# helmholtz-analytics/mpi4torch

Hardware: AMD Instinct MI355X
Metric: allreduce_fwdbwd_algbw_GBps (higher is better)
Workload: dtype bf16; 1 GPU; model=allreduce_1GiB_bf16_fwd_bwd, parallelism=dp1

## Files before the change

csrc/ops.cpp:

```cpp

#include "ops.hpp"
#include "transport.hpp"
#include "kernels.hpp"

#include <torch/csrc/autograd/function.h>
#include <torch/csrc/autograd/functions/utils.h>
#include <torch/csrc/autograd/variable.h>
#include <ATen/core/TensorBody.h>
#include <ATen/WrapDimUtils.h>

#include <ATen/hip/impl/HIPStreamMasqueradingAsCUDA.h>

#include <algorithm>
#include <cstdlib>
#include <cstring>
#include <functional>
#include <limits>
#include <map>
#include <mutex>
#include <tuple>

namespace m4a {

using at::Tensor;
using torch::autograd::Node;
using torch::autograd::variable_list;


Communicator::Communicator(std::string group_name)
    : group_name_(std::move(group_name)) {}

int64_t Communicator::GetRank() { return cpu_tr().rank(); }
int64_t Communicator::GetSize() { return cpu_tr().size(); }

Transport& Communicator::cpu_tr() {
  std::lock_guard<std::mutex> g(mu_);
  if (!cpu_tr_) {
    cpu_tr_ = group_name_.empty() ? make_local_transport()
                                  : make_c10d_transport(group_name_);
  }
  return *cpu_tr_;
}

Transport& Communicator::gpu_tr(int device) {
  std::lock_guard<std::mutex> g(mu_);
  if (!gpu_tr_) {
    if (group_name_.empty()) {
      if (!cpu_tr_) cpu_tr_ = make_local_transport();
      return *cpu_tr_;
    }
    gpu_tr_ = make_rccl_transport(group_name_, device);
    gpu_device_ = device;
  }
  TORCH_CHECK(device == gpu_device_,
              "mpi4torch_amd: one GPU per process (torchrun model); "
              "communicator bound to device ", gpu_device_,
              " but got a tensor on device ", device);
  return *gpu_tr_;
}

Transport& Communicator::tr_for(const Tensor& t) {
  if (t.is_cuda() && !config().force_host_staging) {
    return gpu_tr((int)t.get_device());
  }
  return cpu_tr();
}

namespace {

struct DeviceStager {
  explicit DeviceStager(const Tensor& t)
      : orig_device_(t.device()),
        active_(t.is_cuda() && config().force_host_staging) {}
  Tensor to_comm(const Tensor& t) const {
    return active_ ? t.to(at::kCPU) : t;
  }
  Tensor from_comm(Tensor t) const {
    return active_ ? t.to(orig_device_) : std::move(t);
  }
  at::Device orig_device_;
  bool active_;
};


struct AxisGeom {
  int64_t before = 1, axis = 0, after = 1, after_b = 0, esize = 0;
};

AxisGeom axis_geom(const Tensor& t, int64_t axis) {
  AxisGeom g;
  auto sizes = t.sizes();
  for (int64_t i = 0; i < axis; ++i) g.before *= sizes[i];
  g.axis = sizes[axis];
  for (int64_t i = axis + 1; i < (int64_t)sizes.size(); ++i)
    g.after *= sizes[i];
  g.esize = t.element_size();
  g.after_b = g.after * g.esize;
  return g;
}

hipStream_t current_gpu_stream(const Tensor& t) {
  return c10::hip::getCurrentHIPStreamMasqueradingAsCUDA((int)t.get_device())
      .stream();
}

void move_axis_blocks(const Tensor& full, int64_t axis,
                      const std::vector<int64_t>& displs,
                      const std::vector<int64_t>& counts,
                      std::vector<Tensor>& blocks, bool pack,
                      int64_t row_lo = 0, int64_t row_hi = -1) {
  const auto g = axis_geom(full, axis);
  if (row_hi < 0) row_hi = g.before;
  const int64_t rows = row_hi - row_lo;
  if (rows <= 0) return;
  if (full.is_cuda()) {
    std::vector<SlabDesc> descs;
    descs.reserve(counts.size());
    char* base = static_cast<char*>(full.data_ptr());
    for (size_t i = 0; i < counts.size(); ++i) {
      if (counts[i] == 0 || g.before * g.after == 0) continue;
      char* bp = static_cast<char*>(blocks[i].data_ptr());
      SlabDesc d;
      d.before = rows;
      d.count = counts[i];
      d.after_b = g.after_b;
      if (pack) {
        d.src = base + displs[i] * g.after_b + row_lo * g.axis * g.after_b;
        d.src_pitch_b = g.axis * g.after_b;
        d.dst = bp + row_lo * counts[i] * g.after_b;
        d.dst_pitch_b = counts[i] * g.after_b;
      } else {
        d.src = bp + row_lo * counts[i] * g.after_b;
        d.src_pitch_b = counts[i] * g.after_b;
        d.dst = base + displs[i] * g.after_b + row_lo * g.axis * g.after_b;
        d.dst_pitch_b = g.axis * g.after_b;
      }
      descs.push_back(d);
    }
    if (!descs.empty()) {
      launch_slab_copy(descs.data(), (int)descs.size(),
                       current_gpu_stream(full));
    }
  } else {
    if (g.before * g.after == 0) return;
    auto f3 = full.view({g.before, g.axis, g.after})
                  .narrow(0, row_lo, rows);
    for (size_t i = 0; i < counts.size(); ++i) {
      if (counts[i] == 0) continue;
      auto b3 = blocks[i].view({g.before, counts[i], g.after})
                    .narrow(0, row_lo, rows);
      if (pack) {
        b3.copy_(f3.narrow(1, displs[i], counts[i]));
      } else {
        f3.narrow(1, displs[i], counts[i]).copy_(b3);
      }
    }
  }
}


Tensor fast_clone(const Tensor& in) {
  if (!in.is_cuda() || in.numel() == 0) return in.clone();
  auto out = at::empty_like(in);
  SlabDesc d;
  d.src = in.data_ptr();
  d.dst = out.data_ptr();
  d.before = 1;
  d.count = 1;
  d.after_b = in.numel() * in.element_size();
  d.src_pitch_b = d.after_b;
  d.dst_pitch_b = d.after_b;
  launch_slab_copy(&d, 1, current_gpu_stream(in));
  return out;
}

std::vector<int64_t> prefix_displs(const std::vector<int64_t>& counts) {
  std::vector<int64_t> d(counts.size(), 0);
  for (size_t i = 1; i < counts.size(); ++i) d[i] = d[i - 1] + counts[i - 1];
  return d;
}

int64_t phase_count(const Tensor& t, int64_t per_rank_bytes) {
  const int64_t c = config().pipeline_chunk_bytes;
  if (c <= 0) return 1;
  if (t.is_cuda()) {
    hipStreamCaptureStatus st = hipStreamCaptureStatusNone;
    (void)hipStreamIsCapturing(current_gpu_stream(t), &st);
    if (st != hipStreamCaptureStatusNone) return 1;
  }
  return std::min<int64_t>(
      4, std::max<int64_t>(1, (per_rank_bytes + c - 1) / c));
}

void phased_funnel_exchange(
    Transport& tr, int64_t K, int64_t rows,
    const std::vector<Tensor>& sblocks, const std::vector<int>& speers,
    const std::vector<int64_t>& srowe, std::vector<Tensor>& rblocks,
    const std::vector<int>& rpeers, const std::vector<int64_t>& rrowe,
    const std::function<void(int64_t, int64_t)>& pack_phase,
    const std::function<void(int64_t, int64_t)>& unpack_phase) {
  auto bound = [&](int64_t k) { return rows * k / K; };
  auto slice = [](const Tensor& blk, int64_t lo, int64_t len) {
    auto flat = blk.view({-1});
    return len > 0 ? flat.narrow(0, lo, len) : flat.narrow(0, 0, 0);
  };
  std::vector<uint64_t> reqs((size_t)K);
  for (int64_t k = 0; k < K; ++k) {
    const int64_t b0 = bound(k), b1 = bound(k + 1);
    if (pack_phase) pack_phase(b0, b1);
    std::vector<Tensor> sk(sblocks.size()), rk(rblocks.size());
    for (size_t i = 0; i < sblocks.size(); ++i) {
      sk[i] = slice(sblocks[i], b0 * srowe[i], (b1 - b0) * srowe[i]);
    }
    for (size_t j = 0; j < rblocks.size(); ++j) {
      rk[j] = slice(rblocks[j], b0 * rrowe[j], (b1 - b0) * rrowe[j]);
    }
    reqs[(size_t)k] = tr.iexchange(sk, speers, rk, rpeers);
  }
  for (int64_t k = 0; k < K; ++k) {
    wait_request(reqs[(size_t)k]);
    if (unpack_phase) unpack_phase(bound(k), bound(k + 1));
  }
}


bool is_logical(int64_t op) { return op == kLAnd || op == kLOr || op == kLXor; }
bool is_bitwise(int64_t op) { return op == kBAnd || op == kBOr || op == kBXor; }
bool is_arith(int64_t op) {
  return op == kSum || op == kProd || op == kMin || op == kMax;
}

struct SigHash {
  size_t h;
  explicit SigHash(const char* opname) : h(std::hash<std::string>()(opname)) {}
  void mix(int64_t v) {
    h ^= std::hash<int64_t>()(v) + 0x9e3779b97f4a7c15ull + (h << 6) + (h >> 2);
  }
};

void debug_compare_sig(const std::string& group, const char* opname,
                       SigHash& sig) {
  auto all =
      host_allgather_int64(group, (int64_t)(sig.h & 0x7fffffffffffffffll));
  for (size_t r = 1; r < all.size(); ++r) {
    TORCH_CHECK(all[r] == all[0],
                "mpi4torch_amd[debug]: collective desync detected at ", opname,
                " — rank ", r, " issued a different op/shape/dtype/arguments "
                "than rank 0. This would deadlock without "
                "MPI4TORCH_AMD_DEBUG=1.");
  }
}

void debug_check_collective(const std::string& group, const char* opname,
                            const at::Tensor& t,
                            std::initializer_list<int64_t> args) {
  if (!config().debug_collectives || group.empty()) return;
  SigHash sig(opname);
  sig.mix((int64_t)t.scalar_type());
  for (auto s : t.sizes()) sig.mix(s);
  for (auto a : args) sig.mix(a);
  debug_compare_sig(group, opname, sig);
}

void debug_check_axis_collective(const std::string& group, const char* opname,
                                 const at::Tensor& t,
                                 std::initializer_list<int64_t> axes,
                                 std::initializer_list<int64_t> args) {
  if (!config().debug_collectives || group.empty()) return;
  SigHash sig(opname);
  sig.mix((int64_t)t.scalar_type());
  sig.mix(t.dim());
  for (int64_t i = 0; i < t.dim(); ++i) {
    bool skip = false;
    for (auto a : axes) skip = skip || a == i;
    sig.mix(skip ? -1 : t.size(i));
  }
  for (auto a : args) sig.mix(a);
  debug_compare_sig(group, opname, sig);
}

void debug_check_dtype_collective(const std::string& group,
                                  const char* opname, at::ScalarType dtype,
                                  std::initializer_list<int64_t> args) {
  if (!config().debug_collectives || group.empty()) return;
  SigHash sig(opname);
  sig.mix((int64_t)dtype);
  for (auto a : args) sig.mix(a);
  debug_compare_sig(group, opname, sig);
}

void check_op(int64_t op) {
  TORCH_CHECK(op >= kMax && op <= kMaxLoc, "invalid reduction op ", op);
}

bool is_pairloc(int64_t op) { return op == kMinLoc || op == kMaxLoc; }

bool native_reduce_dtype(const Transport& tr, at::ScalarType t) {
  if (tr.is_gpu()) {
    switch (t) {
      case at::kByte:
      case at::kChar:
      case at::kInt:
      case at::kLong:
      case at::kHalf:
      case at::kFloat:
      case at::kDouble:
      case at::kBFloat16:
        return true;
      case at::kFloat8_e4m3fn:
      case at::kFloat8_e5m2: {
        static const bool want_native = []() {
          const char* e = std::getenv("MPI4TORCH_AMD_NATIVE_FP8");
          return e && e[0] == '1';
        }();
        return want_native &&
               const_cast<Transport&>(tr).fp8_reduce_supported(t);
      }
      default:
        return false;
    }
  }
  switch (t) {
    case at::kByte:
    case at::kChar:
    case at::kInt:
// ... 1765 lines not shown
  }();
  attach_history(result, grad_fn);
  return result;
}


namespace {
struct AlltoallvBackward : public M4ANode {
  AlltoallvBackward(int64_t gaxis, int64_t saxis,
                    std::vector<int64_t> tgt, std::vector<int64_t> src)
      : gaxis(gaxis), saxis(saxis), tgt(std::move(tgt)),
        src(std::move(src)) {}
  std::string name() const override { return "M4AAlltoallvBackward"; }
  variable_list apply(variable_list&& grads) override {
    variable_list out(1);
    if (should_compute_output(0)) {
      out[0] = comm->Alltoallv(grads[0], saxis, gaxis, tgt, src);
    }
    return out;
  }
  int64_t gaxis, saxis;
  std::vector<int64_t> tgt, src;
};

struct AlltoallBackward : public M4ANode {
  AlltoallBackward(int64_t gaxis, int64_t saxis, int64_t numelem)
      : gaxis(gaxis), saxis(saxis), numelem(numelem) {}
  std::string name() const override { return "M4AAlltoallBackward"; }
  variable_list apply(variable_list&& grads) override {
    variable_list out(1);
    if (should_compute_output(0)) {
      out[0] = comm->Alltoall(grads[0], saxis, gaxis, numelem);
    }
    return out;
  }
  int64_t gaxis, saxis, numelem;
};

}

Tensor Communicator::AlltoallvImpl(const Tensor& input, int64_t gatheraxis,
                                   int64_t scatteraxis, int64_t numelem,
                                   const std::vector<int64_t>& target_counts,
                                   const std::vector<int64_t>& source_sizes) {
  gatheraxis = at::maybe_wrap_dim(gatheraxis, input.dim());
  scatteraxis = at::maybe_wrap_dim(scatteraxis, input.dim());
  const bool explicit_counts = !target_counts.empty();
  std::shared_ptr<M4ANode> grad_fn;
  if (torch::autograd::compute_requires_grad(input)) {
    if (explicit_counts) {
      grad_fn = make_node<AlltoallvBackward>(
          c10::intrusive_ptr<Communicator>::unsafe_reclaim_from_nonowning(this),
          gatheraxis, scatteraxis, source_sizes, target_counts);
    } else {
      grad_fn = make_node<AlltoallBackward>(
          c10::intrusive_ptr<Communicator>::unsafe_reclaim_from_nonowning(this),
          gatheraxis, scatteraxis, input.size(gatheraxis));
    }
    grad_fn->set_next_edges(torch::autograd::collect_next_edges(input));
  }
  auto result = [&]() {
    at::AutoDispatchBelowADInplaceOrView guard;
    DeviceStager stager(input);
    auto in = stager.to_comm(input).contiguous().variable_data();
    auto& tr = tr_for(in);
    if (w1_shortcut(tr)) {
      const int64_t want = explicit_counts ? target_counts[0] : numelem;
      TORCH_CHECK(want == in.size(scatteraxis),
                  "Alltoall: numelem must equal the scatter-axis size at "
                  "world size 1");
      return stager.from_comm(fast_clone(in));
    }
    const int me = tr.rank();
    const int P = tr.size();
    debug_check_axis_collective(group_name_, "Alltoall", in,
                                {gatheraxis, scatteraxis},
                                {gatheraxis, scatteraxis, explicit_counts});

    std::vector<int64_t> scounts;
    if (explicit_counts) {
      TORCH_CHECK((int)target_counts.size() == P,
                  "Alltoallv: target_counts must have world_size entries");
      TORCH_CHECK((int)source_sizes.size() == P,
                  "Alltoallv: source_sizes must have world_size entries");
      scounts = target_counts;
    } else {
      scounts = host_allgather_int64(group_name_, numelem);
    }
    auto sdispls = prefix_displs(scounts);

    std::vector<int64_t> s_offs(P), s_lens(P);
    std::vector<int64_t> r_offs(P), r_lens(P);
    std::vector<int64_t> outsizes = in.sizes().vec();
    int64_t send_axis = scatteraxis, recv_axis = gatheraxis;
    std::vector<int64_t> srcsz;

    if (gatheraxis != scatteraxis) {
      const int64_t stotal = sdispls.back() + scounts.back();
      TORCH_CHECK(in.size(scatteraxis) == stotal,
                  "Alltoall: scatter-axis size (", in.size(scatteraxis),
                  ") must equal the sum of per-rank numelem (", stotal, ")");
      auto gsizes = explicit_counts
                        ? source_sizes
                        : host_allgather_int64(group_name_,
                                               in.size(gatheraxis));
      TORCH_CHECK(gsizes[me] == in.size(gatheraxis),
                  "Alltoallv: source_sizes[rank] must equal the local "
                  "gather-axis size");
      auto gdispls = prefix_displs(gsizes);
      for (int j = 0; j < P; ++j) {
        s_offs[j] = sdispls[j];
        s_lens[j] = scounts[j];
        r_offs[j] = gdispls[j];
        r_lens[j] = gsizes[j];
      }
      outsizes[gatheraxis] = gdispls.back() + gsizes.back();
      outsizes[scatteraxis] = scounts[me];
      srcsz = gsizes;
    } else {
      auto nsizes = explicit_counts
                        ? source_sizes
                        : host_allgather_int64(group_name_,
                                               in.size(gatheraxis));
      TORCH_CHECK(nsizes[me] == in.size(gatheraxis),
                  "Alltoallv: source_sizes[rank] must equal the local "
                  "axis size");
      auto ndispls = prefix_displs(nsizes);
      const int64_t totaln = ndispls.back() + nsizes.back();
      const int64_t totalm = sdispls.back() + scounts.back();
      TORCH_CHECK(totaln == totalm,
                  "Alltoall (same axis): global axis length mismatch (",
                  totaln, " vs ", totalm, ")");
      const int64_t my_lo = ndispls[me], my_hi = my_lo + nsizes[me];
      const int64_t tgt_lo = sdispls[me], tgt_hi = tgt_lo + scounts[me];
      for (int j = 0; j < P; ++j) {
        const int64_t slo = std::max(my_lo, sdispls[j]);
        const int64_t shi = std::min(my_hi, sdispls[j] + scounts[j]);
        s_offs[j] = slo - my_lo;
        s_lens[j] = std::max<int64_t>(0, shi - slo);
        const int64_t rlo = std::max(ndispls[j], tgt_lo);
        const int64_t rhi = std::min(ndispls[j] + nsizes[j], tgt_hi);
        r_offs[j] = rlo - tgt_lo;
        r_lens[j] = std::max<int64_t>(0, rhi - rlo);
      }
      outsizes[gatheraxis] = scounts[me];
      srcsz = nsizes;
    }

    auto out = at::empty(outsizes, in.options());
    const auto gs = axis_geom(in, send_axis);
    const auto gr = axis_geom(out, recv_axis);
    const bool send_packed = gs.before != 1;
    const bool recv_packed = gr.before != 1;
    auto sblocks = make_blocks(in, gs.before, gs.after, s_lens, s_offs, &in);
    auto rblocks = make_blocks(out, gr.before, gr.after, r_lens, r_offs, &out);
    auto peers = iota_peers(P);

    int64_t send_before_shared = 1, recv_before_shared = 1;
    {
      const int64_t src_max =
          *std::max_element(srcsz.begin(), srcsz.end());
      const int64_t sc_max =
          *std::max_element(scounts.begin(), scounts.end());
      auto insz = in.sizes();
      for (int64_t d = 0; d < send_axis; ++d) {
        send_before_shared *=
            (d == recv_axis && send_axis != recv_axis) ? src_max : insz[d];
      }
      for (int64_t d = 0; d < recv_axis; ++d) {
        recv_before_shared *= (d == scatteraxis && send_axis != recv_axis)
                                  ? sc_max
                                  : outsizes[d];
      }
    }
    const bool send_m = send_before_shared > 1;
    const bool recv_m = recv_before_shared > 1;
    int64_t K = 1;
    if ((send_m || recv_m) &&
        (send_axis == recv_axis || send_m != recv_m)) {
      int64_t global_elems = 1;
      for (size_t d = 0; d < outsizes.size(); ++d) {
        global_elems *= (d == (size_t)scatteraxis)
                            ? (sdispls.back() + scounts.back())
                            : outsizes[d];
      }
      K = phase_count(in, global_elems / P * in.element_size());
    }

    if (K > 1) {
      const int me_ = me;
      auto send_geom = [&](int j) -> std::pair<int64_t, int64_t> {
        if (send_axis == recv_axis || send_m) {
          return {gs.before, s_lens[j] * gs.after};
        }
        int64_t before = 1, after = 1;
        for (int64_t d = 0; d < (int64_t)outsizes.size(); ++d) {
          const int64_t sz =
              (d == scatteraxis) ? scounts[j] : outsizes[d];
          if (d < recv_axis) before *= sz;
          else if (d > recv_axis) after *= sz;
        }
        return {before, srcsz[me_] * after};
      };
      auto recv_geom = [&](int i) -> std::pair<int64_t, int64_t> {
        if (send_axis == recv_axis || recv_m) {
          return {gr.before, r_lens[i] * gr.after};
        }
        int64_t before = 1, after = 1;
        auto insz = in.sizes();
        for (int64_t d = 0; d < (int64_t)insz.size(); ++d) {
          const int64_t sz = (d == recv_axis) ? srcsz[i] : insz[d];
          if (d < send_axis) before *= sz;
          else if (d > send_axis) after *= sz;
        }
        return {before, scounts[me_] * after};
      };
      auto bound = [&](int64_t rows, int64_t k) { return rows * k / K; };
      auto slice = [](const Tensor& blk, int64_t lo, int64_t len) {
        auto flat = blk.view({-1});
        return len > 0 ? flat.narrow(0, lo, len) : flat.narrow(0, 0, 0);
      };
      std::vector<uint64_t> reqs((size_t)K);
      for (int64_t k = 0; k < K; ++k) {
        if (send_packed) {
          move_axis_blocks(in, send_axis, s_offs, s_lens, sblocks, true,
                           bound(gs.before, k), bound(gs.before, k + 1));
        }
        std::vector<Tensor> sk(P), rk(P);
        for (int j = 0; j < P; ++j) {
          auto sg = send_geom(j);
          sk[j] = slice(sblocks[j], bound(sg.first, k) * sg.second,
                        (bound(sg.first, k + 1) - bound(sg.first, k)) *
                            sg.second);
          auto rg = recv_geom(j);
          rk[j] = slice(rblocks[j], bound(rg.first, k) * rg.second,
                        (bound(rg.first, k + 1) - bound(rg.first, k)) *
                            rg.second);
        }
        reqs[(size_t)k] = tr.iexchange(sk, peers, rk, peers);
      }
      for (int64_t k = 0; k < K; ++k) {
        wait_request(reqs[(size_t)k]);
        if (recv_packed) {
          move_axis_blocks(out, recv_axis, r_offs, r_lens, rblocks, false,
                           bound(gr.before, k), bound(gr.before, k + 1));
        }
      }
      return stager.from_comm(std::move(out));
    }

    if (send_packed) {
      move_axis_blocks(in, send_axis, s_offs, s_lens, sblocks, true);
    }
    tr.exchange(sblocks, peers, rblocks, peers);
    if (recv_packed) {
      move_axis_blocks(out, recv_axis, r_offs, r_lens, rblocks,
                       false);
    }
    return stager.from_comm(std::move(out));
  }();
  attach_history(result, grad_fn);
  return result;
}

Tensor Communicator::Alltoall(const Tensor& input, int64_t gatheraxis,
                              int64_t scatteraxis, int64_t numelem) {
  return AlltoallvImpl(input, gatheraxis, scatteraxis, numelem, {}, {});
}

Tensor Communicator::Alltoallv(const Tensor& input, int64_t gatheraxis,
                               int64_t scatteraxis,
                               std::vector<int64_t> target_counts,
                               std::vector<int64_t> source_sizes) {
  TORCH_CHECK(!target_counts.empty(),
              "Alltoallv: target_counts must not be empty");
  return AlltoallvImpl(input, gatheraxis, scatteraxis,
                       -1, target_counts, source_sizes);
}



namespace {
struct AlltoallPairwiseBackward : public M4ANode {
  AlltoallPairwiseBackward(int64_t axis, std::vector<int64_t> send,
                           std::vector<int64_t> recv)
      : axis(axis), send(std::move(send)), recv(std::move(recv)) {}
  std::string name() const override { return "M4AAlltoallPairwiseBackward"; }
  variable_list apply(variable_list&& grads) override {
    variable_list out(1);
    if (should_compute_output(0)) {
      out[0] = comm->AlltoallPairwise(grads[0], axis, recv, send);
    }
    return out;
  }
  int64_t axis;
  std::vector<int64_t> send, recv;
};
}

Tensor Communicator::AlltoallPairwise(const Tensor& input, int64_t axis,
                                      std::vector<int64_t> send_counts,
                                      std::vector<int64_t> recv_counts) {
  axis = at::maybe_wrap_dim(axis, input.dim());
  auto& tr0 = cpu_tr();
  const int P = tr0.size();
  TORCH_CHECK((int)send_counts.size() == P,
              "AlltoallPairwise: send_counts must have world_size entries");
  if (recv_counts.empty() && P > 1) {
    auto mat = host_allgather_int64_vec(group_name_, send_counts);
    recv_counts.resize(P);
    const int me = tr0.rank();
    for (int j = 0; j < P; ++j) recv_counts[j] = mat[(int64_t)j * P + me];
  }
  if (P == 1 && recv_counts.empty()) recv_counts = send_counts;
  TORCH_CHECK((int)recv_counts.size() == P,
              "AlltoallPairwise: recv_counts must have world_size entries");

  std::shared_ptr<M4ANode> grad_fn;
  if (torch::autograd::compute_requires_grad(input)) {
    grad_fn = make_node<AlltoallPairwiseBackward>(
        c10::intrusive_ptr<Communicator>::unsafe_reclaim_from_nonowning(this),
        axis, send_counts, recv_counts);
    grad_fn->set_next_edges(torch::autograd::collect_next_edges(input));
  }
  auto result = [&]() {
    at::AutoDispatchBelowADInplaceOrView guard;
    DeviceStager stager(input);
    auto in = stager.to_comm(input).contiguous().variable_data();
    auto& tr = tr_for(in);
    auto s_displs = prefix_displs(send_counts);
    auto r_displs = prefix_displs(recv_counts);
    const int64_t s_total = s_displs.back() + send_counts.back();
    const int64_t r_total = r_displs.back() + recv_counts.back();
    TORCH_CHECK(in.size(axis) == s_total,
                "AlltoallPairwise: sum of send_counts (", s_total,
                ") must equal the axis size (", in.size(axis), ")");
    auto outsizes = in.sizes().vec();
    outsizes[axis] = r_total;
    auto out = at::empty(outsizes, in.options());
    if (tr.size() == 1 && !config().force_full_path) {
      out.copy_(in);
      return stager.from_comm(std::move(out));
    }
    debug_check_axis_collective(group_name_, "AlltoallPairwise", in, {axis},
                                {axis});
    const auto g = axis_geom(in, axis);
    auto sblocks = make_blocks(in, g.before, g.after, send_counts, s_displs,
                               &in);
    if (g.before != 1) {
      move_axis_blocks(in, axis, s_displs, send_counts, sblocks,
                       true);
    }
    const auto gr = axis_geom(out, axis);
    auto rblocks = make_blocks(out, gr.before, gr.after, recv_counts,
                               r_displs, &out);
    auto peers = iota_peers(tr.size());
    tr.exchange(sblocks, peers, rblocks, peers);
    if (gr.before != 1) {
      move_axis_blocks(out, axis, r_displs, recv_counts, rblocks,
                       false);
    }
    return stager.from_comm(std::move(out));
  }();
  attach_history(result, grad_fn);
  return result;
}


namespace {
struct AlltoallPairwiseCompressedBackward : public M4ANode {
  AlltoallPairwiseCompressedBackward(int64_t axis, std::vector<int64_t> send,
                                     std::vector<int64_t> recv,
                                     c10::optional<Tensor> send_order,
                                     c10::optional<Tensor> recv_order)
      : axis(axis), send(std::move(send)), recv(std::move(recv)),
        send_order(std::move(send_order)),
        recv_order(std::move(recv_order)) {}
  std::string name() const override {
    return "M4AAlltoallPairwiseCompressedBackward";
  }
  variable_list apply(variable_list&& grads) override {
    variable_list out(1);
    if (should_compute_output(0)) {
      out[0] = comm->AlltoallPairwiseCompressed(grads[0], axis, recv, send,
                                                recv_order, send_order);
    }
    return out;
  }
  int64_t axis;
  std::vector<int64_t> send, recv;
  c10::optional<Tensor> send_order, recv_order;
};

void check_pairwise_order(const char* which,
                          const c10::optional<Tensor>& order, int64_t len,
                          const Tensor& input) {
  if (!order.has_value()) return;
  const Tensor& o = *order;
  TORCH_CHECK(o.dim() == 1 && o.numel() == len,
              "AlltoallPairwiseCompressed: ", which, " must be a 1-D tensor "
              "of length ", len, " (the sum of its counts), got shape ",
              o.sizes());
  TORCH_CHECK(o.scalar_type() == at::kLong,
              "AlltoallPairwiseCompressed: ", which, " must be an int64 "
              "tensor, got ", o.scalar_type());
  TORCH_CHECK(o.device() == input.device(),
              "AlltoallPairwiseCompressed: ", which, " must be on the "
// ... 801 lines not shown
```

csrc/transport.cpp:

```cpp

#include "transport.hpp"

#include <torch/csrc/distributed/c10d/Backend.hpp>
#include <torch/csrc/distributed/c10d/ProcessGroup.hpp>
#include <torch/csrc/distributed/c10d/GroupRegistry.hpp>
#include <torch/csrc/distributed/c10d/Types.hpp>

#include <ATen/hip/HIPContext.h>
#include <ATen/hip/impl/HIPStreamMasqueradingAsCUDA.h>
#include <ATen/hip/impl/HIPCachingAllocatorMasqueradingAsCUDA.h>
#include <ATen/hip/impl/HIPGuardImplMasqueradingAsCUDA.h>

#include <hip/hip_runtime_api.h>
#include <rccl/rccl.h>

#include <atomic>
#include <cstdlib>
#include <cstring>
#include <deque>
#include <map>
#include <mutex>
#include <unordered_map>

namespace m4a {
// ... 4 lines not shown
  const char* ffp = std::getenv("MPI4TORCH_AMD_FORCE_FULL_PATH");
  c.force_full_path = ffp && ffp[0] == '1';
  if (const char* to = std::getenv("MPI4TORCH_AMD_TIMEOUT_S")) {
    c.op_timeout_ms = (int64_t)(std::atof(to) * 1000.0);
  }
  if (const char* pc = std::getenv("MPI4TORCH_AMD_PIPELINE_MB")) {
    c.pipeline_chunk_bytes = (int64_t)(std::atof(pc) * 1048576.0);
  }
  const char* fh = std::getenv("MPI4TORCH_AMD_FORCE_HIERARCHICAL");
  c.force_hierarchical = fh && fh[0] == '1';
  const char* ar = std::getenv("MPI4TORCH_AMD_ALLREDUCE");
  const std::string arv = ar ? ar : "auto";
  TORCH_CHECK(arv == "auto" || arv == "native" || arv == "rccl" || arv.empty(),
              "MPI4TORCH_AMD_ALLREDUCE must be auto, native or rccl, got '",
              arv, "'");
  c.allreduce_engine = arv == "native" ? Config::kAllreduceNative
                       : arv == "rccl" ? Config::kAllreduceRccl
                                       : Config::kAllreduceAuto;
}

Config& config() {
  static Config cfg = []() {
    Config c;
    config_from_env(c);
    return c;
  }();
  return cfg;
}

void reload_config_from_env() { config_from_env(config()); }

#define M4A_HIP_CHECK(expr)                                              \
  do {                                                                   \
    hipError_t _e = (expr);                                              \
    TORCH_CHECK(_e == hipSuccess, "mpi4torch_amd HIP error: ",           \
                hipGetErrorString(_e), " at " __FILE__ ":",              \
                __LINE__);                                               \
  } while (0)

#define M4A_NCCL_CHECK(expr)                                             \
  do {                                                                   \
    ncclResult_t _r = (expr);                                            \
    TORCH_CHECK(_r == ncclSuccess, "mpi4torch_amd RCCL error: ",         \
                ncclGetErrorString(_r), " at " __FILE__ ":", __LINE__);  \
  } while (0)

namespace {


struct Request {
  bool gpu = false;
  bool self_pending = false;
  bool deferred = false;
  std::weak_ptr<Transport> owner;
  hipEvent_t event = nullptr;
  int device = -1;
  c10::intrusive_ptr<c10d::Work> work;
  std::vector<c10::intrusive_ptr<c10d::Work>> works;
  at::Tensor buffer;
  std::vector<at::Tensor> buffers;
  c10::intrusive_ptr<c10d::Work> debug_work;
  at::Tensor debug_meta;
  std::vector<int64_t> debug_expect;
  int debug_peer = -1;
};

struct RequestTable {
  std::mutex mu;
  std::unordered_map<uint64_t, Request> reqs;
  std::atomic<uint64_t> next{1};

  uint64_t add(Request r) {
    uint64_t id = next.fetch_add(1);
    std::lock_guard<std::mutex> g(mu);
    reqs.emplace(id, std::move(r));
    return id;
  }
  Request take(uint64_t id) {
    std::lock_guard<std::mutex> g(mu);
    auto it = reqs.find(id);
    TORCH_CHECK(it != reqs.end(),
                "mpi4torch_amd: unknown or already-waited request id ", id);
    Request r = std::move(it->second);
    reqs.erase(it);
    return r;
  }
  Request* peek(uint64_t id) {
    auto it = reqs.find(id);
    return it == reqs.end() ? nullptr : &it->second;
  }
};

RequestTable& requests() {
  static RequestTable t;
  return t;
}


class EventPool {
 public:
  static EventPool& forDevice(int dev) {
    static std::mutex mu;
    static std::map<int, std::unique_ptr<EventPool>> pools;
    std::lock_guard<std::mutex> g(mu);
    auto& p = pools[dev];
    if (!p) p = std::unique_ptr<EventPool>(new EventPool(dev));
    return *p;
  }
  hipEvent_t acquire() {
    {
      std::lock_guard<std::mutex> g(mu_);
      if (!free_.empty()) {
        hipEvent_t e = free_.back();
        free_.pop_back();
        return e;
      }
    }
    c10::hip::HIPGuardMasqueradingAsCUDA guard(dev_);
    hipEvent_t e;
    M4A_HIP_CHECK(hipEventCreateWithFlags(&e, hipEventDisableTiming));
    return e;
  }
  void release(hipEvent_t e) {
    std::lock_guard<std::mutex> g(mu_);
    free_.push_back(e);
  }

 private:
  explicit EventPool(int dev) : dev_(dev) {}
  int dev_;
  std::mutex mu_;
  std::vector<hipEvent_t> free_;
};


struct SelfMatcher {
  struct Pending {
    uint64_t req_id;
    at::Tensor buf;
    int tag;
  };
  std::mutex mu;
  std::map<int, std::deque<Pending>> sends, recvs;

  static void check_tags(int stag, int rtag) {
    if (!config().debug_collectives) return;
    TORCH_CHECK(stag == rtag,
                "mpi4torch_amd[debug]: self send/recv matched FIFO but with "
                "different tags (send tag ", stag, ", recv tag ", rtag,
                "). Matching is FIFO per (peer, channel); tags do not "
                "reorder it — reorder your posts instead.");
  }

  static void complete_pair(const at::Tensor& src, at::Tensor& dst,
                            uint64_t sreq, uint64_t rreq) {
    dst.copy_(src, true);
    auto& tab = requests();
    std::lock_guard<std::mutex> g(tab.mu);
    for (uint64_t id : {sreq, rreq}) {
      Request* r = tab.peek(id);
      if (!r) continue;
      r->self_pending = false;
      if (src.is_cuda()) {
        r->gpu = true;
        r->device = (int)src.get_device();
        auto cur = c10::hip::getCurrentHIPStreamMasqueradingAsCUDA(r->device);
        r->event = EventPool::forDevice(r->device).acquire();
        M4A_HIP_CHECK(hipEventRecord(r->event, cur.stream()));
      }
    }
  }

  uint64_t isend(const at::Tensor& buf, int tag, Channel ch) {
    Request r;
    r.buffer = buf;
    r.self_pending = true;
    uint64_t id = requests().add(std::move(r));
    std::unique_lock<std::mutex> g(mu);
    auto& rq = recvs[(int)ch];
    if (!rq.empty()) {
      Pending p = rq.front();
      rq.pop_front();
      g.unlock();
      check_tags(tag, p.tag);
      complete_pair(buf, p.buf, id, p.req_id);
    } else {
      sends[(int)ch].push_back({id, buf, tag});
    }
    return id;
  }
  uint64_t irecv(at::Tensor& buf, int tag, Channel ch) {
    Request r;
    r.buffer = buf;
    r.self_pending = true;
    uint64_t id = requests().add(std::move(r));
    std::unique_lock<std::mutex> g(mu);
    auto& sq = sends[(int)ch];
    if (!sq.empty()) {
      Pending p = sq.front();
      sq.pop_front();
      g.unlock();
      check_tags(p.tag, tag);
      complete_pair(p.buf, buf, p.req_id, id);
    } else {
      recvs[(int)ch].push_back({id, buf, tag});
    }
    return id;
  }
};

SelfMatcher& self_matcher() {
  static SelfMatcher m;
  return m;
}


ncclDataType_t nccl_reduce_dtype(at::ScalarType t) {
  switch (t) {
    case at::kByte: return ncclUint8;
    case at::kBool: return ncclUint8;
    case at::kChar: return ncclInt8;
    case at::kInt: return ncclInt32;
    case at::kLong: return ncclInt64;
    case at::kHalf: return ncclFloat16;
    case at::kFloat: return ncclFloat32;
    case at::kDouble: return ncclFloat64;
    case at::kBFloat16: return ncclBfloat16;
    case at::kFloat8_e4m3fn: return ncclFloat8e4m3;
    case at::kFloat8_e5m2: return ncclFloat8e5m2;
    default:
      TORCH_CHECK(false, "mpi4torch_amd: dtype ", t,
                  " not supported for RCCL reductions");
  }
}

ncclRedOp_t nccl_red_op(RedOp op) {
  switch (op) {
    case kSum: return ncclSum;
    case kProd: return ncclProd;
    case kMin: return ncclMin;
    case kMax: return ncclMax;
    default:
      TORCH_CHECK(false, "mpi4torch_amd internal: op ", red_op_name(op),
                  " must be lowered before reaching the RCCL transport");
  }
}

c10d::ReduceOp c10d_red_op(RedOp op) {
  switch (op) {
    case kSum: return c10d::ReduceOp(c10d::ReduceOp::RedOpType::SUM);
    case kProd: return c10d::ReduceOp(c10d::ReduceOp::RedOpType::PRODUCT);
    case kMin: return c10d::ReduceOp(c10d::ReduceOp::RedOpType::MIN);
    case kMax: return c10d::ReduceOp(c10d::ReduceOp::RedOpType::MAX);
    case kBAnd: return c10d::ReduceOp(c10d::ReduceOp::RedOpType::BAND);
    case kBOr: return c10d::ReduceOp(c10d::ReduceOp::RedOpType::BOR);
    case kBXor: return c10d::ReduceOp(c10d::ReduceOp::RedOpType::BXOR);
    default:
      TORCH_CHECK(false, "mpi4torch_amd internal: op ", red_op_name(op),
                  " must be lowered before reaching the c10d transport");
  }
}

void wait_work(const c10::intrusive_ptr<c10d::Work>& w) {
  const int64_t ms = config().op_timeout_ms;
  if (ms > 0) {
    TORCH_CHECK(w->wait(std::chrono::milliseconds(ms)),
                "mpi4torch_amd: collective timed out after ", ms,
                " ms (MPI4TORCH_AMD_TIMEOUT_S) — a peer likely diverged; "
                "run with MPI4TORCH_AMD_DEBUG=1 to locate the desync");
  } else {
    w->wait();
  }
}

c10::intrusive_ptr<c10d::Backend> gloo_backend(const std::string& group_name) {
  auto pg = c10d::resolve_process_group(group_name);
  TORCH_CHECK(pg, "mpi4torch_amd: process group '", group_name,
              "' not found in c10d registry");
  return pg->getBackend(c10::DeviceType::CPU);
}

int chan_tag(Channel ch) { return 1 + (int)ch; }
int meta_tag(Channel ch) { return 16 + (int)ch; }

void attach_debug_handshake(Request& r,
                            const c10::intrusive_ptr<c10d::Backend>& backend,
                            bool is_send, const at::Tensor& buf, int peer,
                            int tag, Channel ch) {
  if (!config().debug_collectives || !backend) return;
  auto meta = at::zeros({3}, at::TensorOptions().dtype(at::kLong));
  std::vector<at::Tensor> ts{meta};
  if (is_send) {
    auto* m = meta.data_ptr<int64_t>();
    m[0] = tag;
    m[1] = (int64_t)buf.scalar_type();
    m[2] = buf.numel();
    r.debug_work = backend->send(ts, peer, meta_tag(ch));
  } else {
    r.debug_expect = {(int64_t)tag, (int64_t)buf.scalar_type(), buf.numel()};
    r.debug_work = backend->recv(ts, peer, meta_tag(ch));
  }
  r.debug_meta = meta;
  r.debug_peer = peer;
}

void check_debug_handshake(Request& r) {
  if (!r.debug_work) return;
  wait_work(r.debug_work);
  if (r.debug_expect.empty()) return;
// ... 238 lines not shown
    std::lock_guard<std::mutex> g(mu_);
    out.copy_(in);
    std::vector<at::Tensor> ts{out};
    c10d::AllreduceOptions opts;
    opts.reduceOp = c10d_red_op(op);
    Request r;
    r.buffer = out;
    r.work = backend_->allreduce(ts, opts);
    return requests().add(std::move(r));
  }
  uint64_t ireduce_scatter(const at::Tensor& in, at::Tensor& out,
                           RedOp op) override {
    reduce_scatter_equal(in, out, op);
    Request r;
    r.buffer = out;
    return requests().add(std::move(r));
  }
  uint64_t iallgather(const at::Tensor& in, at::Tensor& out) override {
    std::lock_guard<std::mutex> g(mu_);
    auto chunks = out.view({size(), -1}).unbind(0);
    std::vector<at::Tensor> outs;
    for (auto& c : chunks) outs.push_back(c.view_as(in));
    std::vector<std::vector<at::Tensor>> outputs{outs};
    std::vector<at::Tensor> inputs{const_cast<at::Tensor&>(in)};
    Request r;
    r.buffer = out;
    r.work = backend_->allgather(outputs, inputs);
    return requests().add(std::move(r));
  }

 private:
  std::string name_;
  c10::intrusive_ptr<c10d::Backend> backend_;
  std::mutex mu_;
};


struct RcclTransport final : Transport {
  RcclTransport(const std::string& group_name, int device)
      : device_(device),
        streams_{c10::hip::getStreamFromPoolMasqueradingAsCUDA(true, device),
                 c10::hip::getStreamFromPoolMasqueradingAsCUDA(true, device),
                 c10::hip::getStreamFromPoolMasqueradingAsCUDA(true, device)} {
    auto backend = gloo_backend(group_name);
    host_backend_ = backend;
    rank_ = backend->getRank();
    size_ = backend->getSize();
    ncclUniqueId ids[3];
    auto idt = at::empty({(int64_t)(3 * sizeof(ncclUniqueId))},
                         at::TensorOptions().dtype(at::kByte));
    if (rank_ == 0) {
      for (auto& id : ids) M4A_NCCL_CHECK(ncclGetUniqueId(&id));
      std::memcpy(idt.data_ptr(), ids, sizeof(ids));
    }
    {
      std::vector<at::Tensor> ts{idt};
      c10d::BroadcastOptions opts;
      opts.rootRank = 0;
      backend->broadcast(ts, opts)->wait();
    }
    std::memcpy(ids, idt.data_ptr(), sizeof(ids));
    M4A_HIP_CHECK(hipSetDevice(device_));
    for (int i = 0; i < 3; ++i) {
      M4A_NCCL_CHECK(ncclCommInitRank(&comms_[i], size_, ids[i], rank_));
    }
  }

  ~RcclTransport() override {
    for (auto& c : comms_) {
      if (c) ncclCommDestroy(c);
    }
  }

  int rank() const override { return rank_; }
  int size() const override { return size_; }
  bool is_gpu() const override { return true; }

  void allreduce(const at::Tensor& in, at::Tensor& out, RedOp op) override {
    std::lock_guard<std::mutex> g(mu_);
    Hop hop(*this, Channel::Coll, {in, out});
    M4A_NCCL_CHECK(ncclAllReduce(in.data_ptr(), out.data_ptr(), in.numel(),
                                 nccl_reduce_dtype(in.scalar_type()),
                                 nccl_red_op(op), comm(Channel::Coll),
                                 hop.stream()));
  }
  void broadcast(at::Tensor& t, int root) override {
    std::lock_guard<std::mutex> g(mu_);
    Hop hop(*this, Channel::Coll, {t});
    M4A_NCCL_CHECK(ncclBroadcast(t.data_ptr(), t.data_ptr(), nbytes(t),
                                 ncclUint8, root, comm(Channel::Coll),
                                 hop.stream()));
  }
  void reduce(at::Tensor& t, RedOp op, int root) override {
    std::lock_guard<std::mutex> g(mu_);
    Hop hop(*this, Channel::Coll, {t});
    M4A_NCCL_CHECK(ncclReduce(t.data_ptr(), t.data_ptr(), t.numel(),
                              nccl_reduce_dtype(t.scalar_type()),
                              nccl_red_op(op), root, comm(Channel::Coll),
                              hop.stream()));
  }
  void allgather_equal(const at::Tensor& in, at::Tensor& out) override {
    std::lock_guard<std::mutex> g(mu_);
    Hop hop(*this, Channel::Coll, {in, out});
    M4A_NCCL_CHECK(ncclAllGather(in.data_ptr(), out.data_ptr(), nbytes(in),
                                 ncclUint8, comm(Channel::Coll),
                                 hop.stream()));
  }
  void reduce_scatter_equal(const at::Tensor& in, at::Tensor& out,
                            RedOp op) override {
    std::lock_guard<std::mutex> g(mu_);
    Hop hop(*this, Channel::Coll, {in, out});
    M4A_NCCL_CHECK(ncclReduceScatter(in.data_ptr(), out.data_ptr(),
                                     out.numel(),
                                     nccl_reduce_dtype(out.scalar_type()),
                                     nccl_red_op(op), comm(Channel::Coll),
                                     hop.stream()));
  }
  void exchange(const std::vector<at::Tensor>& sendbufs,
                const std::vector<int>& speers,
                std::vector<at::Tensor>& recvbufs,
                const std::vector<int>& rpeers) override {
    std::lock_guard<std::mutex> g(mu_);
    std::vector<at::Tensor> all(sendbufs);
    all.insert(all.end(), recvbufs.begin(), recvbufs.end());
    Hop hop(*this, Channel::Coll, all);
    const int me = rank_;
    std::vector<const at::Tensor*> self_sends;
    std::vector<at::Tensor*> self_recvs;
    M4A_NCCL_CHECK(ncclGroupStart());
    for (size_t i = 0; i < sendbufs.size(); ++i) {
      if (speers[i] == me) {
        self_sends.push_back(&sendbufs[i]);
        continue;
      }
      if (nbytes(sendbufs[i]) == 0) continue;
      M4A_NCCL_CHECK(ncclSend(sendbufs[i].data_ptr(), nbytes(sendbufs[i]),
                              ncclUint8, speers[i], comm(Channel::Coll),
                              hop.stream()));
    }
    for (size_t j = 0; j < recvbufs.size(); ++j) {
      if (rpeers[j] == me) {
        self_recvs.push_back(&recvbufs[j]);
        continue;
      }
      if (nbytes(recvbufs[j]) == 0) continue;
      M4A_NCCL_CHECK(ncclRecv(recvbufs[j].data_ptr(), nbytes(recvbufs[j]),
                              ncclUint8, rpeers[j], comm(Channel::Coll),
                              hop.stream()));
    }
    M4A_NCCL_CHECK(ncclGroupEnd());
    TORCH_CHECK(self_sends.size() == self_recvs.size(),
                "exchange: unmatched self blocks");
    for (size_t i = 0; i < self_sends.size(); ++i) {
      M4A_HIP_CHECK(hipMemcpyAsync(
          self_recvs[i]->data_ptr(), self_sends[i]->data_ptr(),
          nbytes(*self_sends[i]), hipMemcpyDeviceToDevice, hop.stream()));
    }
  }
  uint64_t isend(const at::Tensor& buf, int peer, int tag,
                 Channel ch) override {
    if (peer == rank_) return self_matcher().isend(buf, tag, ch);
    std::lock_guard<std::mutex> g(mu_);
    check_not_capturing("Isend");
    return defer_p2p(true, buf, peer, tag, ch);
  }
  uint64_t irecv(at::Tensor& buf, int peer, int tag, Channel ch) override {
    if (peer == rank_) return self_matcher().irecv(buf, tag, ch);
    std::lock_guard<std::mutex> g(mu_);
    check_not_capturing("Irecv");
    return defer_p2p(false, buf, peer, tag, ch);
  }

  void flush_p2p() override {
    std::lock_guard<std::mutex> g(mu_);
    flush_pending_locked();
  }
  uint64_t iexchange(const std::vector<at::Tensor>& sendbufs,
                     const std::vector<int>& speers,
                     std::vector<at::Tensor>& recvbufs,
                     const std::vector<int>& rpeers) override {
    std::lock_guard<std::mutex> g(mu_);
    check_not_capturing("iexchange");
    std::vector<at::Tensor> all(sendbufs);
    all.insert(all.end(), recvbufs.begin(), recvbufs.end());
    enter_side(Channel::Coll, all);
    const int me = rank_;
    std::vector<const at::Tensor*> self_sends;
    std::vector<at::Tensor*> self_recvs;
    M4A_NCCL_CHECK(ncclGroupStart());
    for (size_t i = 0; i < sendbufs.size(); ++i) {
      if (speers[i] == me) {
        self_sends.push_back(&sendbufs[i]);
        continue;
      }
      if (nbytes(sendbufs[i]) == 0) continue;
      M4A_NCCL_CHECK(ncclSend(sendbufs[i].data_ptr(), nbytes(sendbufs[i]),
                              ncclUint8, speers[i], comm(Channel::Coll),
                              stream(Channel::Coll)));
    }
    for (size_t j = 0; j < recvbufs.size(); ++j) {
      if (rpeers[j] == me) {
        self_recvs.push_back(&recvbufs[j]);
        continue;
      }
      if (nbytes(recvbufs[j]) == 0) continue;
      M4A_NCCL_CHECK(ncclRecv(recvbufs[j].data_ptr(), nbytes(recvbufs[j]),
                              ncclUint8, rpeers[j], comm(Channel::Coll),
                              stream(Channel::Coll)));
    }
    M4A_NCCL_CHECK(ncclGroupEnd());
    TORCH_CHECK(self_sends.size() == self_recvs.size(),
                "iexchange: unmatched self blocks");
    for (size_t i = 0; i < self_sends.size(); ++i) {
      M4A_HIP_CHECK(hipMemcpyAsync(
          self_recvs[i]->data_ptr(), self_sends[i]->data_ptr(),
          nbytes(*self_sends[i]), hipMemcpyDeviceToDevice,
          stream(Channel::Coll)));
    }
    uint64_t id = make_gpu_request(Channel::Coll, at::Tensor());
    {
      auto& tab = requests();
      std::lock_guard<std::mutex> tg(tab.mu);
      if (Request* rq = tab.peek(id)) rq->buffers = all;
    }
    return id;
  }
  uint64_t iallgather(const at::Tensor& in, at::Tensor& out) override {
    std::lock_guard<std::mutex> g(mu_);
    check_not_capturing("Iallgather");
    enter_side(Channel::Coll, {in, out});
    M4A_NCCL_CHECK(ncclAllGather(in.data_ptr(), out.data_ptr(), nbytes(in),
                                 ncclUint8, comm(Channel::Coll),
                                 stream(Channel::Coll)));
    return make_gpu_request(Channel::Coll, out);
  }
  uint64_t ireduce_scatter(const at::Tensor& in, at::Tensor& out,
                           RedOp op) override {
    std::lock_guard<std::mutex> g(mu_);
    check_not_capturing("Ireducescatter");
    enter_side(Channel::Coll, {in, out});
    M4A_NCCL_CHECK(ncclReduceScatter(in.data_ptr(), out.data_ptr(),
                                     out.numel(),
                                     nccl_reduce_dtype(out.scalar_type()),
                                     nccl_red_op(op), comm(Channel::Coll),
                                     stream(Channel::Coll)));
    return make_gpu_request(Channel::Coll, out);
  }

  bool fp8_reduce_supported(at::ScalarType t) override {
    const int idx = (t == at::kFloat8_e4m3fn) ? 0 : 1;
    std::lock_guard<std::mutex> g(mu_);
    if (fp8_state_[idx] != 0) return fp8_state_[idx] > 0;
    void* buf = nullptr;
    M4A_HIP_CHECK(hipMalloc(&buf, 64));
    M4A_HIP_CHECK(hipMemsetAsync(buf, 0, 64, stream(Channel::Coll)));
    ncclResult_t rc = ncclAllReduce(
        buf, static_cast<char*>(buf) + 32, 32, nccl_reduce_dtype(t), ncclSum,
        comm(Channel::Coll), stream(Channel::Coll));
    if (rc == ncclSuccess) {
      M4A_HIP_CHECK(hipStreamSynchronize(stream(Channel::Coll)));
    }
    M4A_HIP_CHECK(hipFree(buf));
    fp8_state_[idx] = (rc == ncclSuccess) ? 1 : -1;
    return fp8_state_[idx] > 0;
  }

  uint64_t iallreduce(const at::Tensor& in, at::Tensor& out,
                      RedOp op) override {
    std::lock_guard<std::mutex> g(mu_);
    check_not_capturing("Iallreduce");
    enter_side(Channel::Coll, {in, out});
    M4A_NCCL_CHECK(ncclAllReduce(in.data_ptr(), out.data_ptr(), in.numel(),
                                 nccl_reduce_dtype(in.scalar_type()),
                                 nccl_red_op(op), comm(Channel::Coll),
                                 stream(Channel::Coll)));
    return make_gpu_request(Channel::Coll, out);
  }

 private:
  static size_t nbytes(const at::Tensor& t) {
    return (size_t)t.numel() * t.element_size();
  }
  ncclComm_t comm(Channel ch) { return comms_[(int)ch]; }
  hipStream_t stream(Channel ch) { return streams_[(int)ch].stream(); }

  static bool stream_capturing(hipStream_t s) {
    hipStreamCaptureStatus st = hipStreamCaptureStatusNone;
    (void)hipStreamIsCapturing(s, &st);
    return st != hipStreamCaptureStatusNone;
  }

  void check_not_capturing(const char* what) {
    auto cur = c10::hip::getCurrentHIPStreamMasqueradingAsCUDA(device_);
    TORCH_CHECK(!stream_capturing(cur.stream()),
                "mpi4torch_amd: ", what,
                " inside hipGraph capture is not supported (its Wait may "
                "fall outside the graph); capture blocking collectives only");
  }

  void check_async_errors() {
    for (int i = 0; i < 3; ++i) {
      if (!comms_[i]) continue;
      ncclResult_t async_err = ncclSuccess;
      if (ncclCommGetAsyncError(comms_[i], &async_err) == ncclSuccess) {
        TORCH_CHECK(async_err == ncclSuccess || async_err == ncclInProgress,
                    "mpi4torch_amd: RCCL communicator (channel ", i,
                    ") is in an error state: ",
                    ncclGetErrorString(async_err),
                    " — a peer likely failed; restart the job");
      }
    }
  }

  void enter_side(Channel ch, const std::vector<at::Tensor>& tensors) {
    check_async_errors();
    auto cur = c10::hip::getCurrentHIPStreamMasqueradingAsCUDA(device_);
    auto& pool = EventPool::forDevice(device_);
    hipEvent_t e = pool.acquire();
    M4A_HIP_CHECK(hipEventRecord(e, cur.stream()));
    M4A_HIP_CHECK(hipStreamWaitEvent(stream(ch), e, 0));
    pool.release(e);
    for (const auto& t : tensors) {
      c10::hip::HIPCachingAllocatorMasqueradingAsCUDA::
          recordStreamMasqueradingAsCUDA(t.storage().data_ptr(),
                                         streams_[(int)ch]);
    }
  }
  void exit_side(Channel ch) {
    auto cur = c10::hip::getCurrentHIPStreamMasqueradingAsCUDA(device_);
    auto& pool = EventPool::forDevice(device_);
    hipEvent_t e = pool.acquire();
    M4A_HIP_CHECK(hipEventRecord(e, stream(ch)));
    M4A_HIP_CHECK(hipStreamWaitEvent(cur.stream(), e, 0));
    pool.release(e);
  }
  uint64_t make_gpu_request(Channel ch, const at::Tensor& buf) {
    Request r;
    r.gpu = true;
    r.device = device_;
    r.event = EventPool::forDevice(device_).acquire();
    M4A_HIP_CHECK(hipEventRecord(r.event, stream(ch)));
    r.buffer = buf;
    return requests().add(std::move(r));
  }

  struct PendingP2P {
    bool is_send;
    at::Tensor buf;
    int peer;
    Channel ch;
    uint64_t req_id;
    hipEvent_t ready;
  };

  uint64_t defer_p2p(bool is_send, const at::Tensor& buf, int peer, int tag,
                     Channel ch) {
    check_async_errors();
    auto cur = c10::hip::getCurrentHIPStreamMasqueradingAsCUDA(device_);
    auto& pool = EventPool::forDevice(device_);
    hipEvent_t ready = pool.acquire();
    M4A_HIP_CHECK(hipEventRecord(ready, cur.stream()));
    c10::hip::HIPCachingAllocatorMasqueradingAsCUDA::
        recordStreamMasqueradingAsCUDA(buf.storage().data_ptr(),
                                       streams_[(int)ch]);
    Request r;
    r.gpu = true;
    r.device = device_;
    r.deferred = true;
    r.buffer = buf;
    r.owner = weak_from_this();
    attach_debug_handshake(r, host_backend_, is_send, buf, peer, tag, ch);
    uint64_t id = requests().add(std::move(r));
    pending_.push_back({is_send, buf, peer, ch, id, ready});
    return id;
  }

  void flush_pending_locked() {
    if (pending_.empty()) return;
    check_async_errors();
    auto& pool = EventPool::forDevice(device_);
    for (auto& p : pending_) {
      M4A_HIP_CHECK(hipStreamWaitEvent(stream(p.ch), p.ready, 0));
      pool.release(p.ready);
    }
    M4A_NCCL_CHECK(ncclGroupStart());
    for (auto& p : pending_) {
      if (nbytes(p.buf) == 0) continue;
      if (p.is_send) {
        M4A_NCCL_CHECK(ncclSend(p.buf.data_ptr(), nbytes(p.buf), ncclUint8,
                                p.peer, comm(p.ch), stream(p.ch)));
      } else {
        M4A_NCCL_CHECK(ncclRecv(p.buf.data_ptr(), nbytes(p.buf), ncclUint8,
                                p.peer, comm(p.ch), stream(p.ch)));
      }
    }
    M4A_NCCL_CHECK(ncclGroupEnd());
    auto& tab = requests();
    std::lock_guard<std::mutex> tg(tab.mu);
    for (auto& p : pending_) {
      Request* r = tab.peek(p.req_id);
      if (!r) continue;
      r->deferred = false;
      r->event = pool.acquire();
      M4A_HIP_CHECK(hipEventRecord(r->event, stream(p.ch)));
    }
    pending_.clear();
  }

  struct Hop {
    Hop(RcclTransport& t, Channel ch, const std::vector<at::Tensor>& ts)
        : t_(t), ch_(ch) {
      auto cur = c10::hip::getCurrentHIPStreamMasqueradingAsCUDA(t_.device_);
      capturing_ = stream_capturing(cur.stream());
      if (capturing_) {
        use_stream_ = cur.stream();
      } else {
        t_.enter_side(ch_, ts);
        use_stream_ = t_.stream(ch_);
      }
    }
    ~Hop() {
      if (!capturing_) t_.exit_side(ch_);
    }
    hipStream_t stream() const { return use_stream_; }
    RcclTransport& t_;
    Channel ch_;
    hipStream_t use_stream_;
    bool capturing_ = false;
  };

  int device_;
  int rank_ = 0, size_ = 1;
  std::mutex mu_;
  ncclComm_t comms_[3] = {nullptr, nullptr, nullptr};
  int fp8_state_[2] = {0, 0};
  c10::hip::HIPStreamMasqueradingAsCUDA streams_[3];
  c10::intrusive_ptr<c10d::Backend> host_backend_;
  std::vector<PendingP2P> pending_;
};

}

void wait_request(uint64_t id) {
  {
    std::shared_ptr<Transport> owner;
    {
      auto& tab = requests();
      std::lock_guard<std::mutex> g(tab.mu);
      Request* r = tab.peek(id);
      TORCH_CHECK(r, "mpi4torch_amd: unknown or already-waited request id ",
                  id);
      if (r->deferred) owner = r->owner.lock();
    }
    if (owner) owner->flush_p2p();
  }
  Request r = requests().take(id);
  TORCH_CHECK(!r.self_pending,
              "mpi4torch_amd: Wait() on a self send/recv whose matching "
              "operation was never posted");
  TORCH_CHECK(!r.deferred,
              "mpi4torch_amd internal: deferred p2p request not flushed");
  if (!r.debug_expect.empty()) check_debug_handshake(r);
  if (r.gpu) {
    auto cur = c10::hip::getCurrentHIPStreamMasqueradingAsCUDA(r.device);
    M4A_HIP_CHECK(hipStreamWaitEvent(cur.stream(), r.event, 0));
    EventPool::forDevice(r.device).release(r.event);
  } else if (r.work) {
    wait_work(r.work);
  }
  for (auto& w : r.works) wait_work(w);
  if (r.debug_expect.empty()) check_debug_handshake(r);
}

std::shared_ptr<Transport> make_local_transport() {
  return std::make_shared<LocalTransport>();
}

std::shared_ptr<Transport> make_c10d_transport(const std::string& group_name) {
  return std::make_shared<C10dTransport>(group_name);
}

std::shared_ptr<Transport> make_rccl_transport(const std::string& group_name,
                                               int device) {
  return std::make_shared<RcclTransport>(group_name, device);
}

std::vector<int64_t> host_allgather_int64(const std::string& group_name,
                                          int64_t value) {
  auto backend = gloo_backend(group_name);
  const int n = backend->getSize();
  auto in = at::full({1}, value, at::TensorOptions().dtype(at::kLong));
  auto out = at::empty({n}, at::TensorOptions().dtype(at::kLong));
  std::vector<at::Tensor> outs;
  outs.reserve(n);
  for (int i = 0; i < n; ++i) outs.push_back(out[i].view({1}));
  std::vector<std::vector<at::Tensor>> outputs{outs};
  std::vector<at::Tensor> inputs{in};
  backend->allgather(outputs, inputs)->wait();
  std::vector<int64_t> res(n);
  std::memcpy(res.data(), out.data_ptr(), n * sizeof(int64_t));
  return res;
}

std::vector<int64_t> host_allgather_int64_vec(
    const std::string& group_name, const std::vector<int64_t>& v) {
  auto backend = gloo_backend(group_name);
  const int n = backend->getSize();
  const int64_t len = (int64_t)v.size();
  auto in = at::empty({len}, at::TensorOptions().dtype(at::kLong));
  std::memcpy(in.data_ptr(), v.data(), len * sizeof(int64_t));
  auto out = at::empty({n * len}, at::TensorOptions().dtype(at::kLong));
  std::vector<at::Tensor> outs;
  outs.reserve(n);
  for (int i = 0; i < n; ++i) outs.push_back(out.narrow(0, i * len, len));
  std::vector<std::vector<at::Tensor>> outputs{outs};
  std::vector<at::Tensor> inputs{in};
  backend->allgather(outputs, inputs)->wait();
  std::vector<int64_t> res(n * len);
  std::memcpy(res.data(), out.data_ptr(), n * len * sizeof(int64_t));
  return res;
}

std::vector<int64_t> host_broadcast_int64(const std::string& group_name,
                                          const std::vector<int64_t>& values,
                                          int root, int64_t fixed_len) {
  auto backend = gloo_backend(group_name);
  int64_t len = fixed_len;
  if (len < 0) {
    auto lt = at::full({1}, (int64_t)values.size(),
                       at::TensorOptions().dtype(at::kLong));
    std::vector<at::Tensor> ts{lt};
    c10d::BroadcastOptions opts;
    opts.rootRank = root;
    backend->broadcast(ts, opts)->wait();
    len = lt.item<int64_t>();
  }
  auto t = at::zeros({len}, at::TensorOptions().dtype(at::kLong));
  if (backend->getRank() == root) {
    TORCH_CHECK((int64_t)values.size() == len);
    std::memcpy(t.data_ptr(), values.data(), len * sizeof(int64_t));
  }
  std::vector<at::Tensor> ts{t};
  c10d::BroadcastOptions opts;
  opts.rootRank = root;
  backend->broadcast(ts, opts)->wait();
  std::vector<int64_t> res(len);
  std::memcpy(res.data(), t.data_ptr(), len * sizeof(int64_t));
  return res;
}

}
```

Baseline: 3143 GB/s.

## Route self-copies through arithmetic copy kernel and bypass transport for own block

Replaces the slab-copy and hipMemcpyAsync device-to-device paths for fast_clone, self-matched send/recv completion and self blocks in exchange with a compute-kernel copy (launch_arith_copy) when buffers do not overlap. In alltoallv, the rank's own block is copied directly, or aliased into the pack/unpack buffer, instead of going through the transport exchange. The aim is to avoid DMA-engine memcpy overhead and an extra staging hop for local data. It adds more branching and aliasing logic, and the new kernel may not beat hipMemcpy for large sizes.

```diff
diff --git a/csrc/ops.cpp b/csrc/ops.cpp
--- a/csrc/ops.cpp
+++ b/csrc/ops.cpp
@@ -162,15 +162,8 @@
 Tensor fast_clone(const Tensor& in) {
   if (!in.is_cuda() || in.numel() == 0) return in.clone();
   auto out = at::empty_like(in);
-  SlabDesc d;
-  d.src = in.data_ptr();
-  d.dst = out.data_ptr();
-  d.before = 1;
-  d.count = 1;
-  d.after_b = in.numel() * in.element_size();
-  d.src_pitch_b = d.after_b;
-  d.dst_pitch_b = d.after_b;
-  launch_slab_copy(&d, 1, current_gpu_stream(in));
+  launch_arith_copy(in.data_ptr(), out.data_ptr(),
+                    in.numel() * in.element_size(), current_gpu_stream(in));
   return out;
 }
 
@@ -2242,9 +2235,44 @@
     const auto gr = axis_geom(out, recv_axis);
     const bool send_packed = gs.before != 1;
     const bool recv_packed = gr.before != 1;
-    auto sblocks = make_blocks(in, gs.before, gs.after, s_lens, s_offs, &in);
-    auto rblocks = make_blocks(out, gr.before, gr.after, r_lens, r_offs, &out);
-    auto peers = iota_peers(P);
+    const bool own_direct = !(send_packed && recv_packed);
+    auto without_own = [&](std::vector<int64_t> lens) {
+      if (own_direct) lens[(size_t)me] = 0;
+      return lens;
+    };
+    auto sblocks = make_blocks(in, gs.before, gs.after,
+                               send_packed ? without_own(s_lens) : s_lens,
+                               s_offs, &in);
+    auto rblocks = make_blocks(out, gr.before, gr.after,
+                               recv_packed ? without_own(r_lens) : r_lens,
+                               r_offs, &out);
+    std::vector<int> peers;
+    for (int j = 0; j < P; ++j) {
+      if (!(own_direct && j == me)) peers.push_back(j);
+    }
+    auto wire = [&](const std::vector<Tensor>& blocks) {
+      std::vector<Tensor> w;
+      w.reserve(peers.size());
+      for (int j : peers) w.push_back(blocks[(size_t)j]);
+      return w;
+    };
+    if (own_direct) {
+      if (send_packed) {
+        sblocks[(size_t)me] = rblocks[(size_t)me];
+      } else if (recv_packed) {
+        rblocks[(size_t)me] = sblocks[(size_t)me];
+      } else if (sblocks[(size_t)me].numel() > 0) {
+        auto& s = sblocks[(size_t)me];
+        auto& r = rblocks[(size_t)me];
+        if (in.is_cuda()) {
+          launch_arith_copy(s.data_ptr(), r.data_ptr(),
+                            s.numel() * s.element_size(),
+                            current_gpu_stream(in));
+        } else {
+          r.copy_(s);
+        }
+      }
+    }
 
     int64_t send_before_shared = 1, recv_before_shared = 1;
     {
@@ -2310,29 +2338,40 @@
         auto flat = blk.view({-1});
         return len > 0 ? flat.narrow(0, lo, len) : flat.narrow(0, 0, 0);
       };
+      const auto s_ph = without_own(s_lens), r_ph = without_own(r_lens);
+      if (own_direct) {
+        std::vector<int64_t> own(P, 0);
+        if (send_packed) {
+          own[(size_t)me] = s_lens[(size_t)me];
+          move_axis_blocks(in, send_axis, s_offs, own, sblocks, true);
+        } else if (recv_packed) {
+          own[(size_t)me] = r_lens[(size_t)me];
+          move_axis_blocks(out, recv_axis, r_offs, own, rblocks, false);
+        }
+      }
       std::vector<uint64_t> reqs((size_t)K);
       for (int64_t k = 0; k < K; ++k) {
         if (send_packed) {
-          move_axis_blocks(in, send_axis, s_offs, s_lens, sblocks, true,
+          move_axis_blocks(in, send_axis, s_offs, s_ph, sblocks, true,
                            bound(gs.before, k), bound(gs.before, k + 1));
         }
-        std::vector<Tensor> sk(P), rk(P);
-        for (int j = 0; j < P; ++j) {
+        std::vector<Tensor> sk, rk;
+        for (int j : peers) {
           auto sg = send_geom(j);
-          sk[j] = slice(sblocks[j], bound(sg.first, k) * sg.second,
-                        (bound(sg.first, k + 1) - bound(sg.first, k)) *
-                            sg.second);
+          sk.push_back(slice(sblocks[j], bound(sg.first, k) * sg.second,
+                             (bound(sg.first, k + 1) - bound(sg.first, k)) *
+                                 sg.second));
           auto rg = recv_geom(j);
-          rk[j] = slice(rblocks[j], bound(rg.first, k) * rg.second,
-                        (bound(rg.first, k + 1) - bound(rg.first, k)) *
-                            rg.second);
+          rk.push_back(slice(rblocks[j], bound(rg.first, k) * rg.second,
+                             (bound(rg.first, k + 1) - bound(rg.first, k)) *
+                                 rg.second));
         }
-        reqs[(size_t)k] = tr.iexchange(sk, peers, rk, peers);
+        if (!peers.empty()) reqs[(size_t)k] = tr.iexchange(sk, peers, rk, peers);
       }
       for (int64_t k = 0; k < K; ++k) {
-        wait_request(reqs[(size_t)k]);
+        if (!peers.empty()) wait_request(reqs[(size_t)k]);
         if (recv_packed) {
-          move_axis_blocks(out, recv_axis, r_offs, r_lens, rblocks, false,
+          move_axis_blocks(out, recv_axis, r_offs, r_ph, rblocks, false,
                            bound(gr.before, k), bound(gr.before, k + 1));
         }
       }
@@ -2342,7 +2381,10 @@
     if (send_packed) {
       move_axis_blocks(in, send_axis, s_offs, s_lens, sblocks, true);
     }
-    tr.exchange(sblocks, peers, rblocks, peers);
+    if (!peers.empty()) {
+      auto sw = wire(sblocks), rw = wire(rblocks);
+      tr.exchange(sw, peers, rw, peers);
+    }
     if (recv_packed) {
       move_axis_blocks(out, recv_axis, r_offs, r_lens, rblocks,
                        false);
diff --git a/csrc/transport.cpp b/csrc/transport.cpp
--- a/csrc/transport.cpp
+++ b/csrc/transport.cpp
@@ -180,9 +180,32 @@
                 "reorder it — reorder your posts instead.");
   }
 
+  static bool is_plain_gpu_copy(const at::Tensor& src, const at::Tensor& dst) {
+    if (!src.is_cuda() || !dst.is_cuda() || src.device() != dst.device())
+      return false;
+    if (src.scalar_type() != dst.scalar_type() || src.sizes() != dst.sizes())
+      return false;
+    if (!src.is_contiguous() || !dst.is_contiguous()) return false;
+    if (src.is_conj() != dst.is_conj() || src.is_neg() != dst.is_neg())
+      return false;
+    const auto n = (uintptr_t)src.numel() * src.element_size();
+    const auto s = reinterpret_cast<uintptr_t>(src.data_ptr());
+    const auto d = reinterpret_cast<uintptr_t>(dst.data_ptr());
+    return s + n <= d || d + n <= s;
+  }
+
   static void complete_pair(const at::Tensor& src, at::Tensor& dst,
                             uint64_t sreq, uint64_t rreq) {
-    dst.copy_(src, true);
+    if (is_plain_gpu_copy(src, dst)) {
+      c10::hip::HIPGuardMasqueradingAsCUDA guard(src.device());
+      launch_arith_copy(
+          src.data_ptr(), dst.data_ptr(),
+          (int64_t)src.numel() * src.element_size(),
+          c10::hip::getCurrentHIPStreamMasqueradingAsCUDA(
+              (int)src.get_device()).stream());
+    } else {
+      dst.copy_(src, true);
+    }
     auto& tab = requests();
     std::lock_guard<std::mutex> g(tab.mu);
     for (uint64_t id : {sreq, rreq}) {
@@ -727,9 +750,7 @@
     TORCH_CHECK(self_sends.size() == self_recvs.size(),
                 "exchange: unmatched self blocks");
     for (size_t i = 0; i < self_sends.size(); ++i) {
-      M4A_HIP_CHECK(hipMemcpyAsync(
-          self_recvs[i]->data_ptr(), self_sends[i]->data_ptr(),
-          nbytes(*self_sends[i]), hipMemcpyDeviceToDevice, hop.stream()));
+      self_copy(*self_sends[i], *self_recvs[i], hop.stream());
     }
   }
   uint64_t isend(const at::Tensor& buf, int peer, int tag,
@@ -787,10 +808,7 @@
     TORCH_CHECK(self_sends.size() == self_recvs.size(),
                 "iexchange: unmatched self blocks");
     for (size_t i = 0; i < self_sends.size(); ++i) {
-      M4A_HIP_CHECK(hipMemcpyAsync(
-          self_recvs[i]->data_ptr(), self_sends[i]->data_ptr(),
-          nbytes(*self_sends[i]), hipMemcpyDeviceToDevice,
-          stream(Channel::Coll)));
+      self_copy(*self_sends[i], *self_recvs[i], stream(Channel::Coll));
     }
     uint64_t id = make_gpu_request(Channel::Coll, at::Tensor());
     {
@@ -982,6 +1000,20 @@
     pending_.clear();
   }
 
+  void self_copy(const at::Tensor& src, at::Tensor& dst, hipStream_t s) {
+    const size_t n = nbytes(src);
+    if (n == 0) return;
+    const auto sp = reinterpret_cast<uintptr_t>(src.data_ptr());
+    const auto dp = reinterpret_cast<uintptr_t>(dst.data_ptr());
+    if (sp + n <= dp || dp + n <= sp) {
+      c10::hip::HIPGuardMasqueradingAsCUDA guard(device_);
+      launch_arith_copy(src.data_ptr(), dst.data_ptr(), (int64_t)n, s);
+    } else {
+      M4A_HIP_CHECK(hipMemcpyAsync(dst.data_ptr(), src.data_ptr(), n,
+                                   hipMemcpyDeviceToDevice, s));
+    }
+  }
+
   struct Hop {
     Hop(RcclTransport& t, Channel ch, const std::vector<at::Tensor>& ts)
         : t_(t), ch_(ch) {
```

Result: no change. 3129 GB/s (median of 2 runs) (-0.4%).
